# thu-nics/ViDiT-Q

Measured on AMD Instinct MI355X. Metric: denoising steps/sec (whole node), OpenSORA STDiT 16x512x512 W8A8, higher is better.
Workload: dtype int8 (W8A8 Linear, int32 acc) + fp16 attention/residual; 1 GPU; OpenSORA STDiT-XL/2 16x512x512 W8A8 (w8a8_dynamic.yaml), 1 prompt per GPU, DDIM-100 schedule, cfg 4.0, cfg_split, depth 28; prompts_in_flight=1, prompts=1, status_word=0, hip_graph=True, cond_uncond_streams=2

## Files before the change

include/viditq.h:

```cpp
#ifndef VIDITQ_H
#define VIDITQ_H

#include <stdint.h>

#ifdef __cplusplus
extern "C" {
#endif

#define VQ_OK 0
#define VQ_EINVAL (-1)
#define VQ_ESHAPE (-2)
#define VQ_ELAUNCH (-3)
#define VQ_EUNSUP (-4)

#define VQ_ST_EPSFILL 1

#define VQ_GEMM_DEFAULT (-1)

#define VQ_EPI_NONE 0
#define VQ_EPI_GELU 1
#define VQ_EPI_GATE_RESID 2
#define VQ_EPI_RESID 3

int vq_version(void);
// ... 187 lines not shown
                     int row, int n_rows, int eps_f16, int xm_f16, void* stream);

#define VQ_SA_ROW 16
#define VQ_SA_CFG 0
#define VQ_SA_SIGMA 1
#define VQ_SA_ALPHA 2
#define VQ_SA_OC 3
#define VQ_SA_CX 4
#define VQ_SA_CG0 5
#define VQ_SA_CG1 6
#define VQ_SA_CN 7
#define VQ_SA_OP 8
#define VQ_SA_PX 9
#define VQ_SA_PG0 10
#define VQ_SA_PG1 11
#define VQ_SA_PN 12
#define VQ_SA_T_NEXT 14
int vq_cfg_sa_step(const void* eps, const float* x, const float* xp, float* hist, const float* noise, const float* coef,
                   const int32_t* step, float* x_out, float* xp_out, void* x_model, int n, int C, int inner, long ld_eps,
                   int row, int n_rows, int eps_f16, int xm_f16, void* stream);

int vq_linear_f16(const void* x, const void* w, const void* bias, void* out, int M, int N, int K, long ldx, long ldw,
                  long ldo, int act_in, int act_out, void* stream);

#ifdef __cplusplus
}
#endif
#endif
```

vidit-q_amd/_lib.py:

```python
from __future__ import annotations

import ctypes as C
import os

_HERE = os.path.dirname(os.path.abspath(__file__))
LIB_PATH = os.environ.get("VIDITQ_LIB") or os.path.join(_HERE, "csrc", "libviditq_hip.so")

VQ_OK = 0
VQ_ST_EPSFILL = 1
EPI_NONE, EPI_GELU, EPI_GATE_RESID, EPI_RESID = 0, 1, 2, 3

_vp, _i, _f, _l = C.c_void_p, C.c_int, C.c_float, C.c_long

SIGNATURES = {
    "vq_version": (_i, []),
    "vq_strerror": (C.c_char_p, [_i]),
    "vq_last_hip_error": (_i, []),
    "vq_gelu_rowquant": (_i, [_vp, _vp, _vp, _vp, _vp, _vp, _vp, _i, _i, _i, _i, _i, _vp, _vp]),
    "vq_rowquant": (_i, [_vp, _vp, _i, _i, _vp, _vp, _vp, _vp, _vp, _vp, _vp, _vp, _vp, _i,
                         _i, _i, _i, _i, _i, _vp, _vp]),
    "vq_ln_modulate_rowquant": (_i, [_vp, _vp, _vp, _f, _i, _vp, _vp, _vp, _vp, _vp, _vp, _vp,
                                     _i, _i, _i, _i, _i, _vp, _vp]),
    "vq_smooth_reciprocal": (_i, [_vp, _vp, _i, _vp, _vp]),
    "vq_rowquant_smooth_multi": (_i, [_vp, _i, _vp, _vp, _vp, _vp, _vp, _vp, _i, _i, _i, _i, _vp, _vp]),
# ... 4 lines not shown
    "vq_smooth_div_check": (_i, [_vp, _vp, _vp, _vp, _l, _vp]),
    "vq_fakequant_act": (_i, [_vp, _vp, _vp, _vp, _vp, _vp, _vp, _i, _i, _i, _i, _i, _i, _vp, _vp, _vp]),
    "vq_epsfill_fixup": (_i, [_vp, _vp, _vp, _vp, _vp, _vp, _i, _i, _i, _i, _i, _vp]),
    "vq_pack_weight": (_i, [_vp, _vp, _vp, _vp, _vp, _vp, _vp, _vp, _i, _i, _i, _i, _vp]),
    "vq_weight_minmax": (_i, [_vp, _vp, _vp, _vp, _i, _i, _i, _i, _vp, _vp]),
    "vq_gemm_i8_batched": (_i, [_vp] * 10 + [_i] * 6 + [_vp]),
    "vq_gemm_i8_grouped": (_i, [_i] + [_vp] * 10 + [_i] * 6 + [_vp]),
    "vq_gemm_i8": (_i, [_vp, _vp, _vp, _vp, _vp, _vp, _vp, _vp, _vp, _vp, _i, _vp, _vp,
                        _i, _i, _i, _i, _i, _i, _i, _i, _vp]),
    "vq_gemm_i8_rowquant_static": (_i, [_vp] * 17 + [_i] * 8 + [_vp]),
    "vq_gemm_i8_cross_attn": (_i, [_vp] * 12 + [_i] * 10 + [_l] * 4 + [_vp, _f, _vp]),
    "vq_gemm_i8_stamped": (_i, [_vp] * 10 + [_i] * 5 + [_vp, _l, _vp]),
    "vq_attn_fwd": (_i, [_vp, _vp, _vp, _vp, _i, _i, _i, _i, _i, _l, _l, _l, _l, _l, _l, _vp, _f, _vp]),
    "vq_attn_fwd_route": (_i, [_vp, _vp, _vp, _vp, _i, _i, _i, _i, _i, _l, _l, _l, _l, _l, _l, _vp, _f, _vp]),
    "vq_attn_temporal": (_i, [_vp, _vp, _vp, _vp, _i, _i, _i, _i, _i, _l, _l, _f, _vp]),
    "vq_attn_temporal_rowquant": (_i, [_vp, _vp, _vp, _vp, _vp, _vp, _vp, _vp, _vp, _vp, _vp, _i, _i, _i, _i, _i, _l, _i, _f,
                                       _vp]),
    "vq_attn_temporal_rowquant_shared": (_i, [_vp] * 11 + [_i] * 5 + [_l, _i, _i, _f, _vp]),
    "vq_attn_temporal_long": (_i, [_vp] * 11 + [_i] * 5 + [_l, _l, _i, _f, _vp]),
    "vq_attn_temporal_rowquant_static": (_i, [_vp] * 12 + [_i] * 5 + [_l, _l, _i, _i, _f, _vp]),
    "vq_attn_fwd_rowquant_static": (_i, [_vp] * 12 + [_i] * 5 + [_l] * 6 + [_vp, _i, _i, _f, _vp]),
    "vq_adaln_table": (_i, [_vp, _vp, _vp, _i, _i, _i, _vp]),
    "vq_linear_f16": (_i, [_vp, _vp, _vp, _vp, _i, _i, _i, _l, _l, _l, _i, _i, _vp]),
    "vq_cfg_ddim_step": (_i, [_vp, _vp, _vp, _vp, _i, _i, _i, _f, _f, _f, _f, _f, _vp]),
    "vq_cfg_dpmpp_step": (_i, [_vp] * 7 + [_i, _i, _i, _l, _i, _i, _i, _i, _vp]),
    "vq_cfg_dpmpp_step_patch": (_i, [_vp] * 8 + [_i] * 9 + [_l] + [_i] * 5 + [_vp]),
    "vq_dpmpp_advance": (_i, [_vp, _vp, _i, _vp, _i, _vp]),
    "vq_cfg_ddpm_step": (_i, [_vp] * 8 + [_i, _i, _i, _l, _i, _i, _i, _i, _i, _vp]),
    "vq_cfg_sa_step": (_i, [_vp] * 10 + [_i, _i, _i, _l, _i, _i, _i, _i, _vp]),
}

DPMPP_ROW = 16
(DPMPP_ORDER, DPMPP_TAYLOR, DPMPP_CFG, DPMPP_SIGMA, DPMPP_ALPHA, DPMPP_INV_ALPHA, DPMPP_X, DPMPP_M0, DPMPP_D1, DPMPP_D2,
 DPMPP_INV_R0, DPMPP_INV_R1, DPMPP_R0_FRAC, DPMPP_INV_R01, DPMPP_T_NEXT) = range(15)
DDPM_ROW = 16
(DDPM_CFG, DDPM_A, DDPM_B, DDPM_C1, DDPM_C2, DDPM_MIN_LOG, DDPM_MAX_LOG, DDPM_NONZERO, DDPM_CLIP) = range(9)
DDPM_T_NEXT = 14
SA_ROW = 16
(SA_CFG, SA_SIGMA, SA_ALPHA, SA_OC, SA_CX, SA_CG0, SA_CG1, SA_CN, SA_OP, SA_PX, SA_PG0, SA_PG1, SA_PN) = range(13)
SA_T_NEXT = 14

_lib = None


class VQError(RuntimeError):
    pass
# ... 36 lines not shown
```

vidit-q_amd/csrc/fp_linear.hip:

```cpp
#include "vq_common.h"

#define FPL_NONE 0
#define FPL_SILU 1
#define FPL_GELU 2

template <int ACT>
__device__ __forceinline__ float fpl_act(float v) {
    if constexpr (ACT == FPL_SILU) {
        return v * __builtin_amdgcn_rcpf(1.0f + __builtin_amdgcn_exp2f(-1.4426950408889634f * v));
    } else if constexpr (ACT == FPL_GELU) {
        const float w = v * fmaf(v * v, -0.044715f * 2.302208198f, -2.302208198f);
        return v * __builtin_amdgcn_rcpf(1.0f + __builtin_amdgcn_exp2f(w));
    } else {
        return v;
    }
}

template <int ACT_IN, int ACT_OUT, bool SPLITK>
__global__ __launch_bounds__(256) void fp_linear_kernel(const half_t* __restrict__ x, const half_t* __restrict__ w,
                                                        const half_t* __restrict__ bias, half_t* __restrict__ out, int M,
                                                        int N, int K, long ldx, long ldw, long ldo) {
    __shared__ float red[3][64][4];
    const int lane = threadIdx.x & 63, wave = __builtin_amdgcn_readfirstlane(threadIdx.x >> 6);
    const int lq = lane & 15, g4 = lane >> 4;
// ... 22 lines not shown
            }
            acc = __builtin_amdgcn_mfma_f32_16x16x32_f16(wa[u], xa[u], acc, 0, 0, 0);
        }
    }
    if constexpr (SPLITK) {
        if (wave > 0) *reinterpret_cast<float4v*>(&red[wave - 1][lane][0]) = acc;
        __syncthreads();
        if (wave > 0) return;
#pragma unroll
        for (int p = 0; p < 3; ++p) {
            const float4v o = *reinterpret_cast<const float4v*>(&red[p][lane][0]);
            acc += o;
        }
    }
    const int m = m0 + lq, n = n0 + 4 * g4;
    if (m < M && n < N) {
        half4 o;
#pragma unroll
        for (int r = 0; r < 4; ++r) o[r] = (half_t)fpl_act<ACT_OUT>(acc[r] + (bias ? (float)bias[n + r] : 0.f));
        *reinterpret_cast<half4*>(out + (long)m * ldo + n) = o;
    }
}

template <int AI, int AO>
static void fpl_go(const half_t* x, const half_t* w, const half_t* bias, half_t* out, int M, int N, int K, long ldx, long ldw,
                   long ldo, hipStream_t st) {
    const int mt = (M + 15) / 16, nt = (N + 15) / 16;
    if (K <= 32)
        hipLaunchKernelGGL((fp_linear_kernel<AI, AO, false>), dim3((mt + 3) / 4, nt), dim3(256), 0, st, x, w, bias, out, M, N, K, ldx,
                           ldw, ldo);
    else
        hipLaunchKernelGGL((fp_linear_kernel<AI, AO, true>), dim3(mt, nt), dim3(256), 0, st, x, w, bias, out, M, N, K, ldx, ldw, ldo);
}

extern "C" int vq_linear_f16(const void* x, const void* w, const void* bias, void* out, int M, int N, int K, long ldx,
                             long ldw, long ldo, int act_in, int act_out, void* stream) {
    if (!x || !w || !out) return VQ_EINVAL;
    if (M <= 0 || N <= 0 || K <= 0) return VQ_EINVAL;
    if (K % 8 != 0 || N % 4 != 0 || ldx % 8 != 0 || ldw % 8 != 0 || ldo % 4 != 0 || ldx < K || ldw < K || ldo < N) return VQ_ESHAPE;
    if (act_in < 0 || act_in > 2 || act_out < 0 || act_out > 2) return VQ_EUNSUP;
    if ((M + 15) / 16 > 2147483647 / 4 || (N + 15) / 16 > 65535) return VQ_ESHAPE;
    const half_t* X = (const half_t*)x;
    const half_t* W = (const half_t*)w;
    const half_t* Bv = (const half_t*)bias;
    half_t* O = (half_t*)out;
    hipStream_t st = (hipStream_t)stream;
#define FPL_CASE(AI, AO) \
    if (act_in == AI && act_out == AO) fpl_go<AI, AO>(X, W, Bv, O, M, N, K, ldx, ldw, ldo, st)
    FPL_CASE(FPL_NONE, FPL_NONE);
    else FPL_CASE(FPL_NONE, FPL_SILU);
    else FPL_CASE(FPL_NONE, FPL_GELU);
    else FPL_CASE(FPL_SILU, FPL_NONE);
    else return VQ_EUNSUP;
#undef FPL_CASE
    return vq_check_launch();
}
```

vidit-q_amd/graph.py:

```python
from __future__ import annotations

import os
from typing import Dict, Hashable, Optional, Tuple

import torch


def _capture(fn, warmup: int, first=None, debug: bool = False):
    side = torch.cuda.Stream()
    side.wait_stream(torch.cuda.current_stream())
    with torch.cuda.stream(side), torch.no_grad():
        if first is not None:
            first()
            side.synchronize()
        for _ in range(warmup):
            fn()
        side.synchronize()
    torch.cuda.current_stream().wait_stream(side)
    graph = torch.cuda.CUDAGraph()
    if debug:
        graph.enable_debug_mode()
    with torch.no_grad(), torch.cuda.graph(graph, capture_error_mode="thread_local"):
        out = fn()
    return graph, out
# ... 12 lines not shown
        self.mask = mask
        self.cfg_split = bool(getattr(qnn, "cfg_split", False))
        from . import _lib
        dump = os.environ.get("VQ_GRAPH_DUMP")

        def counted():
            calls0 = _lib.CALLS[0]
            out = self._forward(timestep_id)
            self.c_abi_calls = _lib.CALLS[0] - calls0
            return out

        self.graph, (self.cond, self.uncond) = _capture(counted, warmup, debug=bool(dump),
                                                        first=lambda: self._forward(timestep_id, serial=True))
        self.dot_path = None
        if dump:
            try:
                self.dot_path = "%s.%d.dot" % (dump, id(self))
                self.graph.debug_dump(self.dot_path)
            except Exception:
                self.dot_path = None

    def _forward(self, t_id, serial=False):
        q = self.qnn
        if self.cfg_split and self.two_streams and not serial:
            cur = torch.cuda.current_stream()
            self.side.wait_stream(cur)
            with torch.cuda.stream(self.side):
                unc = q(self.x, self.t, self.yu, mask=self.mask, timestep_id=t_id)
            cond = q(self.x, self.t, self.yc, mask=self.mask, timestep_id=t_id)
            cur.wait_stream(self.side)
            return cond, unc
        if self.cfg_split:
            return (q(self.x, self.t, self.yc, mask=self.mask, timestep_id=t_id),
                    q(self.x, self.t, self.yu, mask=self.mask, timestep_id=t_id))
        n = self.x.shape[0]
        out = q(torch.cat([self.x, self.x]), torch.cat([self.t, self.t]), torch.cat([self.yc, self.yu]),
                mask=self.mask, timestep_id=t_id)
        return out[:n], out[n:]

    def run(self, x: torch.Tensor, timestep_id: int):
        self.x.copy_(x)
        self.t.fill_(int(timestep_id))
        self.graph.replay()
        return self.cond, self.uncond


# ... 280 lines not shown
```

vidit-q_amd/ops.py:

```python
from __future__ import annotations

import ctypes as C
from dataclasses import dataclass
from typing import List, Optional, Sequence

import torch

from . import _lib
from ._lib import EPI_GATE_RESID, EPI_GELU, EPI_NONE, EPI_RESID, VQError, check


def _L():
    return _lib.load()


def _stream() -> int:
    return torch.cuda.current_stream().cuda_stream


def _p(t: Optional[torch.Tensor]):
    return None if t is None else t.data_ptr()


def _req(t: torch.Tensor, dtype, name: str):
# ... 866 lines not shown
    R = torch.empty(rows, dtype=torch.int32, device=dev)
    scale = float(D) ** -0.5 if scale is None else float(scale)
    check(_L().vq_attn_fwd_rowquant_static(_p(q), _p(k), _p(v), _p(s), _p(s_rcp), _p(delta), _p(zp), _p(xq), _p(sx), _p(zx),
                                           _p(R), _p(o), n_seq, Lq, Lk, H, D, q_seq_stride, q_tok_stride, kv_seq_stride,
                                           kv_tok_stride, o_seq_stride, o_tok_stride, _p(kv_off), Kp, n_bits, scale,
                                           _stream()), "vq_attn_fwd_rowquant_static")
    return QAct(xq, sx, zx, R, Cc, n_bits)


def adaln_table(table: torch.Tensor, t0: torch.Tensor) -> torch.Tensor:
    _req(table, torch.float16, "table")
    _req(t0, torch.float16, "t0")
    J, Cc = table.shape
    B = t0.shape[0]
    assert t0.numel() == B * J * Cc
    mod = torch.empty((J, B, Cc), dtype=torch.float32, device=table.device)
    check(_L().vq_adaln_table(_p(table), _p(t0), _p(mod), B, J, Cc, _stream()), "vq_adaln_table")
    return mod


ACT_NONE, ACT_SILU, ACT_GELU = 0, 1, 2


def linear_f16(x: torch.Tensor, w: torch.Tensor, bias: Optional[torch.Tensor] = None, act_in: int = ACT_NONE,
               act_out: int = ACT_NONE) -> torch.Tensor:
    _req_rows(x, torch.float16, "x")
    _req_rows(w, torch.float16, "w")
    K = x.shape[-1]
    N = w.shape[0]
    assert w.dim() == 2 and w.shape[1] == K and w.stride(1) == 1
    x2 = x.reshape(-1, K)
    if x2.stride(1) != 1:
        x2 = x2.contiguous()
    if bias is not None:
        _req(bias, torch.float16, "bias")
        assert bias.numel() == N and bias.is_contiguous()
    M = x2.shape[0]
    out = torch.empty((M, N), dtype=torch.float16, device=x.device)
    check(_L().vq_linear_f16(_p(x2), _p(w), _p(bias), _p(out), M, N, K, x2.stride(0), w.stride(0), N, act_in, act_out,
                             _stream()), "vq_linear_f16")
    return out.reshape(*x.shape[:-1], N)


def cfg_ddim_step(cond: torch.Tensor, uncond: torch.Tensor, x: torch.Tensor, cfg: float, one_plus_k: float,
                  A: float, Bc: float, abar_prev: float, out: Optional[torch.Tensor] = None) -> torch.Tensor:
    _req(cond, torch.float32, "cond")
    _req(uncond, torch.float32, "uncond")
    _req(x, torch.float32, "x")
    n, Cc = x.shape[0], x.shape[1]
    inner = x[0, 0].numel()
    assert cond.shape[0] == n and cond.shape[1] == 2 * Cc and cond.shape == uncond.shape
    if out is None:
        out = torch.empty_like(x)
    check(_L().vq_cfg_ddim_step(_p(cond), _p(uncond), _p(x), _p(out), n, Cc, inner, float(cfg), float(one_plus_k),
                                float(A), float(Bc), float(abar_prev), _stream()), "vq_cfg_ddim_step")
    return out


def _dense_strides(shape):
    out, acc = [], 1
    for d in reversed(shape):
        out.append(acc)
        acc *= int(d)
    return tuple(reversed(out))
# ... 203 lines not shown
```

vidit-q_amd/qdiff/models/quant_model.py:

```python
from __future__ import annotations

import logging
import warnings

import torch
import torch.nn as nn

from ..quantizer.base_quantizer import ActQuantizer, BaseQuantizer, StraightThrough, WeightQuantizer
from .dit_quant_layer import QuantAttnLinearImg, QuantCrossAttnLinearImg
from .quant_block import BaseQuantBlock, get_specials
from .quant_layer import QuantLayer
from .stdit_quant_layer import QuantCrossAttnLinear, QuantSpatialAttnLinear, QuantTemporalAttnLinear

logger = logging.getLogger(__name__)


def pattern_in(text, pattern):
    patterns = pattern.split(".")
    texts = text.split(".")
    for i in range(len(texts)):
        for j in range(len(patterns)):
            if i + j >= len(texts):
                break
            if patterns[j] == "*":
# ... 213 lines not shown
            return 0
        v = int(self._status.item())
        if v & 1:
            msg = ("a dynamically quantized activation had a token with quant step < 1e-6: the reference would set "
                   "EVERY token's step to 1e-6 here (base_quantizer.py:220-222) and saturate the layer; the integer "
                   "path does not reproduce that degenerate fill - outputs of this run differ from the reference")
            if raise_on_eps:
                raise RuntimeError(msg)
            warnings.warn(msg)
        return v

    def forward(self, x, t, y, timestep_id=None, **kwargs):
        if timestep_id is None:
            timestep_id = t[0].item() if isinstance(t, torch.Tensor) else t
        if self.timestep_wise:
            self.set_timestep_for_quantizer(timestep_id)
        if timestep_id != self._cur_t:
            self.set_timestep_id_for_quantlayer(timestep_id)
            self._cur_t = timestep_id
        if x.is_cuda:
            self.status_word()
        return self.model(x, t, y, **kwargs)

    def __getattr__(self, name):
        try:
            return super().__getattr__(name)
        except AttributeError:
            return getattr(self.model, name)


def _device_of(model):
    for p in model.parameters():
        return p.device
    return torch.device("cpu")
```

vidit-q_amd/t2v/dpm_solver.py:

```python
from __future__ import annotations

from functools import partial

import torch

from ..t2i.dpm_solver import DPMSolverPP, _switch
from .iddpm import _accepts_timestep_id, model_forward_pair

_T2V_DPM_FUSED = _switch("VQ_T2V_DPM_FUSED", False)


def lower_order_final(steps: int) -> bool:
    return steps < 10


def forward_with_dpmsolver(model, x, timestep, y, **kwargs):
    return model.forward(x, timestep, y, **kwargs).chunk(2, dim=1)[0]


class VideoDPMSolverPP(DPMSolverPP):

    def __init__(self, net, condition, uncondition, cfg_scale, model_kwargs=None, cfg_split=False):
        super().__init__(partial(forward_with_dpmsolver, net), condition, uncondition, cfg_scale, model_kwargs)
        self.net, self.cfg_split = net, bool(cfg_split)
# ... 6 lines not shown
            self.model_kwargs["timestep_id"] = t_val
        if not self.cfg_split or self.cfg_scale == 1.0 or self.uncondition is None:
            return super()._noise(x, t_cont)
        t = torch.full((x.shape[0],), t_val, dtype=torch.float32, device=x.device)
        extra = {k: v for k, v in self.model_kwargs.items() if k not in ("mask", "timestep_id")}
        cond, uncond = model_forward_pair(self.net, x, t, self.condition, self.uncondition, self.model_kwargs.get("mask"),
                                          True, t_val, extra)
        return self._guide(torch.cat([uncond.chunk(2, dim=1)[0], cond.chunk(2, dim=1)[0]]))

    def _fused_wanted(self, x, method, fused):
        if fused is None:
            fused = _T2V_DPM_FUSED
        return bool(fused) and method == "multistep" and self.cfg_scale != 1.0 and self.uncondition is not None and x.is_cuda

    def _forward_patch(self, xm, t, t_val, side=None):
        kw = {k: v for k, v in self.model_kwargs.items() if k != "timestep_id"}
        if self._takes_id:
            kw["timestep_id"] = t_val
        net = self.net
        if not self.cfg_split:
            n = xm.shape[0] // 2
            out = net.forward(xm, t, self._joint_text(), patch_major=True, **kw)
            return out[:n], out[n:]
        if side is None:
            eps_c = net.forward(xm, t, self.condition, patch_major=True, **kw)
            return net.forward(xm, t, self.uncondition, patch_major=True, **kw), eps_c
        cur = torch.cuda.current_stream()
        side.wait_stream(cur)
        with torch.cuda.stream(side):
            eps_u = net.forward(xm, t, self.uncondition, patch_major=True, **kw)
        eps_c = net.forward(xm, t, self.condition, patch_major=True, **kw)
        cur.wait_stream(side)
        return eps_u, eps_c

    def _eager_eps(self, pair):
        return torch.cat([self.net.unpatchify(e).to(torch.float32).chunk(2, dim=1)[0] for e in pair])

    def _multistep_fused(self, x, ts, args, step_callback):
        from .. import ops
        from ..t2i.fused_loop import device_table, fused_loop
        n, steps, order = x.shape[0], args[0], args[1]
        copies = 1 if self.cfg_split else 2
        patch = tuple(self.net.patch_size)
        x = x.float().contiguous() if x.dtype != torch.float32 or not x.is_contiguous() else x
        xm = torch.cat([x] * copies).to(self.model_input_dtype)
        hist = torch.empty((3, x.numel()), dtype=torch.float32, device=x.device)
# ... 67 lines not shown
```

vidit-q_amd/t2v/stdit.py:

```python
from __future__ import annotations

import os
from typing import List

import numpy as np
import torch
import torch.nn as nn
import torch.nn.functional as F

from .. import ops
from ..qdiff.models.quant_block import QuantAttention
from ..qdiff.models.quant_layer import QuantLayer
from ..qdiff.quantizer.dynamic_quantizer import DynamicActQuantizer


def approx_gelu():
    return nn.GELU(approximate="tanh")


def t2i_modulate(x, shift, scale):
    return x * (1 + scale) + shift


def get_1d_sincos_pos_embed_from_grid(embed_dim, pos):
# ... 258 lines not shown
        q = self.q_linear(x).reshape(B * N, C).half().contiguous()
        kv = self.kv_linear(cond).reshape(-1, 2 * C).half().contiguous()
        lens = mask if mask is not None else [kv.shape[0] // B] * B
        off = seq_offsets(lens, x.device)
        o = self.core.cross(q, kv, off, B, N)
        return self.proj(o.reshape(B, N, C).to(dt))


def _switch(name: str, default: bool) -> bool:
    return os.environ.get(name, "1" if default else "0") != "0"


_ATTN_QUANT = _switch("VQ_ATTN_QUANT", True)
_GELU_QUANT = _switch("VQ_GELU_QUANT", True)
_STATIC_FUSED = True
_ATTN_QUANT_JOINT = _switch("VQ_ATTN_QUANT_JOINT", False)
_SMOOTH_JOINT = _switch("VQ_SMOOTH_JOINT", False)
_STATIC_ATTN_QUANT = _switch("VQ_STATIC_ATTN_QUANT", False)
_STATIC_FWD_ATTN_QUANT = _switch("VQ_STATIC_FWD_ATTN_QUANT", False)
_STATIC_GEMM_QUANT = _switch("VQ_STATIC_GEMM_QUANT", False)
_RUNNING_SMOOTH_DEVICE = _switch("VQ_RUNNING_SMOOTH_DEVICE", False)
EXACT_KV_EPS_FILL = _switch("VQ_EXACT_KV_EPS_FILL", True)
_CROSS_Q_FUSED = _switch("VQ_CROSS_Q_FUSED", True)


def _tensorwise_static(aq) -> bool:
    return not isinstance(aq, DynamicActQuantizer) and aq.delta.numel() == 1 and aq.zero_point.numel() == 1


def _same_dynamic(layers) -> bool:
    aqs = [l.act_quantizer for l in layers]
    return all(isinstance(a, DynamicActQuantizer) for a in aqs) and len({a.n_bits for a in aqs}) == 1


def _smooth_joint(layers, svs, B, add_rows=False) -> bool:
    return _SMOOTH_JOINT and B == 2 and not add_rows and all(s is not None for s in svs) and _same_dynamic(layers)


def _static_attn_quant(proj, T, H, D) -> bool:
    aq = proj.act_quantizer
    return _STATIC_ATTN_QUANT and _STATIC_FUSED and _tensorwise_static(aq) and ops.attn_temporal_static_ok(
        T, H, D, ops.pad128(H * D), aq.n_bits)


def _static_fwd_attn_quant(proj) -> bool:
    return _STATIC_FWD_ATTN_QUANT and _STATIC_FUSED and _tensorwise_static(proj.act_quantizer)
# ... 28 lines not shown
    aq = proj.act_quantizer
    return fused_call(aq.delta.float(), aq.zero_point.float(), aq.n_bits, sv)


def fused_rules(block, running=False) -> bool:
    for m in block.hot_layers():
        if not (isinstance(m, QuantLayer) and m.int_route_ok()):
            return False
        aq = m.act_quantizer
        if not isinstance(aq, DynamicActQuantizer) and aq.per_group:
            return False
        if getattr(m, "smooth_quant_running_stat", False) and not (
                running and m is block.mlp.fc2 and m.running_stat_device_ok()):
            return False
    return True


def fused_running_rules(block) -> bool:
    return fused_rules(block, running=True)


def takes_fused(block) -> bool:
    return block.fused_ok() or (_RUNNING_SMOOTH_DEVICE and block.fused_running_ok())


def _svec(layer):
    r, alpha = layer._range_and_alpha()
    return layer.smooth_vector(r, alpha)


def _range_of(layer, r):
    return layer._range_and_alpha()[0] if r is None else r


def ln_quant(x3, shift, scale, layers, svs, status):
    l0 = layers[0]
    if len(layers) > 1 and _smooth_joint(layers, svs, x3.shape[0]):
        qas = ops.rowquant_multi_shared(x3, svs, n_bits=l0.act_quantizer.n_bits, status=status, shift=shift, scale=scale,
                                        eps=1e-6)
        if qas is not None:
            return qas
    if all(isinstance(l.act_quantizer, DynamicActQuantizer) for l in layers):
        smooth = [None] if all(s is None for s in svs) else list(svs)
        return ops.ln_modulate_rowquant(x3, shift, scale, 1e-6, smooth=smooth, n_bits=l0.act_quantizer.n_bits,
                                        status=status)
    if _static_one_pass(layers, x3.shape[-1], ln=True):
# ... 13 lines not shown
            return qas
    if all(s is None for s in svs) and isinstance(aq, DynamicActQuantizer):
        return [att.q.quantize_input(x3, None, add_rows=tpe2, add_div=S)]
    if tpe2 is None and B == 1 and all(s is not None for s in svs) and _same_dynamic(layers):
        return ops.rowquant_multi(x3, svs, n_bits=aq.n_bits, status=st)
    if _static_one_pass(layers, x3.shape[-1], add_rows=tpe2 is not None):
        delta, zp = _static_grids(layers)
        return ops.rowquant_static(x3, delta, zp, n_bits=aq.n_bits, smooth=svs, add_rows=tpe2, add_div=S)
    return [l.quantize_input(x3, s, add_rows=tpe2, add_div=S) for l, s in zip(layers, svs)]


def temporal_proj_codes(att, qkv, B, T, S, sv):
    proj, aq = att.proj, att.proj.act_quantizer
    dynamic = isinstance(aq, DynamicActQuantizer)
    if _ATTN_QUANT and dynamic and aq.n_bits == 8 and (B == 1 or not _ATTN_QUANT_JOINT):
        return att.core.temporal_quantized(qkv, B, T, S, status=proj.status, s=sv)
    if _ATTN_QUANT and _ATTN_QUANT_JOINT and dynamic:
        return att.core.temporal_quantized_shared(qkv, B, T, S, aq.n_bits, status=proj.status, s=sv)
    if _static_attn_quant(proj, T, att.core.num_heads, att.core.head_dim):
        return att.core.temporal_quantized_static(qkv, B, T, S, aq.delta.float(), aq.zero_point.float(), aq.n_bits, s=sv)
    return None


def proj_into_resid(layer, r, qa, x2, gate=None, rows_per_gate=None, pw=None):
    if pw is None:
        pw = layer.packed_weight(_range_of(layer, r), _svec(layer))
    if gate is None:
        return ops.gemm_i8(qa, pw, bias=layer.bias_f32(), out=x2, epilogue=ops.EPI_RESID, resid=x2)
    return ops.gemm_i8(qa, pw, bias=layer.bias_f32(), out=x2, epilogue=ops.EPI_GATE_RESID, resid=x2, gate=gate,
                       rows_per_gate=rows_per_gate)


def attn_proj_stage(proj, r, x2, B, N, fused, plain, att_o, gate=None):
    sv = _svec(proj)
    qa = fused(sv)
    if qa is None:
        att_o = plain(att_o)
        qa = proj.quantize_input(att_o.view(B, N, -1), sv)
    proj_into_resid(proj, r, qa, x2, gate, N)
    return att_o


def _cross_q_fused_shape(H, D, K, B, N, bound=None) -> bool:
    C, Kp = H * D, (K + 127) // 128 * 128
    return D == 72 and C % 288 == 0 and N > 0 and N % 256 == 0 and 0 < K <= 16384 and B * N * Kp < 1 << 32 and \
        C * Kp < 1 << 32 and (bound is None or 0 < bound <= 128)


_CROSS_Q_FUSED_ROUND = 256


def _cross_q_fused(ca, B, N) -> bool:
    H, D = ca.core.num_heads, ca.core.head_dim
    return _CROSS_Q_FUSED and not _static_fwd_attn_quant(ca.proj) and _cross_q_fused_shape(
        H, D, ca.q_linear.in_features, B, N) and ((B * N // 256) * (H * D // 288)) % _CROSS_Q_FUSED_ROUND == 0


def cross_stage(ca, r, x2, x3, B, N, y_lens, prompt_kv, att_o):
    ql, sv = ca.q_linear, _svec(ca.q_linear)
    kv = None
    if _cross_q_fused(ca, B, N):
        kv = prompt_kv()
        core = ca.core
        C = core.num_heads * core.head_dim
        bound = int(getattr(y_lens, "max_len", 0)) or kv.shape[0]
        if _cross_q_fused_shape(core.num_heads, core.head_dim, ql.in_features, B, N, bound) and kv.stride(0) % 8 == 0:
            def fused_q(o):
                if o is None:
                    o = torch.empty((B * N, C), dtype=torch.float16, device=x3.device)
                return ops.gemm_i8_cross_attn(ql.quantize_input(x3, sv), ql.packed_weight(_range_of(ql, r), sv), ql.bias_f32(),
                                              kv, kv[:, C:], o, B, N, bound, core.num_heads, core.head_dim, 0, kv.stride(0),
                                              N * o.stride(0), o.stride(0), kv_off=y_lens, scale=core.scale)
            return attn_proj_stage(ca.proj, r, x2, B, N, lambda s: None, fused_q, att_o)
    q = ops.gemm_i8(ql.quantize_input(x3, sv), ql.packed_weight(_range_of(ql, r), sv), bias=ql.bias_f32())
    if kv is None:
        kv = prompt_kv()
    return attn_proj_stage(
        ca.proj, r, x2, B, N,
        lambda s: fwd_attn_quantized_static(ca.proj, s, lambda d, z, nb, sm: ca.core.cross_quantized_static(
            q, kv, y_lens, B, N, d, z, nb, s=sm)),
        lambda o: ca.core.cross(q, kv, y_lens, B, N, out=o), att_o)


def mlp_stage(mlp, r, x2, x3, B, N, shift, scale, gate, status):
    fc1, fc2 = mlp.fc1, mlp.fc2
    s1 = _svec(fc1)
    qa = ln_quant(x3, shift, scale, (fc1,), [s1], status)[0]
    pw1 = fc1.packed_weight(_range_of(fc1, r), s1)
    if getattr(fc2, "smooth_quant_running_stat", False):
        h = ops.gemm_i8(qa, pw1, bias=fc1.bias_f32(), epilogue=ops.EPI_GELU)
        qa, pw2 = fc2.running_stat_step(h.view(B, N, -1))
        return proj_into_resid(fc2, r, qa, x2, gate, N, pw=pw2)
    s2 = _svec(fc2)
    qa2 = mlp_quantized_static(fc1, fc2, qa, pw1, s2)
    if qa2 is None:
        one_pass = _GELU_QUANT and fc2.gelu_one_pass_ok(B, fc2.in_features, s2)
        h = ops.gemm_i8(qa, pw1, bias=fc1.bias_f32(), epilogue=ops.EPI_NONE if one_pass else ops.EPI_GELU)
        h3 = h.view(B, N, -1)
        qa2 = fc2.quantize_gelu_input(h3, s2) if one_pass else fc2.quantize_input(h3, s2)
    return proj_into_resid(fc2, r, qa2, x2, gate, N)


def prompt_kv_exact_fill(layer, y3, r, sv, pw):
    aq = layer.act_quantizer
# ... 99 lines not shown
        kkey = (y2, pw_kv.wq, ca.kv_linear.act_quantizer.n_bits)
        kv = self._kv_cache.get(kkey) if self.cache_prompt else None
        if kv is None:
            kv = prompt_kv_exact_fill(ca.kv_linear, y2.view(1, -1, C), r, sv, pw_kv)
            if self.cache_prompt:
                self._kv_cache.put(kkey, kv)
        return kv

    def _qkv_gemm(self, att, r, svs, qas, M):
        layers = (att.q, att.k, att.v)
        fused, pws = self._qkv_weights(att, r, svs)
        C = self.hidden_size
        qkv = torch.empty((M, 3 * C), dtype=torch.float16, device=qas[0].xq.device)
        if fused is not None and len(qas) == 1:
            ops.gemm_i8(qas[0], fused[0], bias=fused[1], out=qkv)
        elif len({(p.N, p.K, p.Kp, p.n_bits) for p in pws}) == 1 and len({(a.K, a.Kp) for a in qas}) == 1:
            ops.gemm_i8_grouped([qas[j if len(qas) > 1 else 0] for j in range(3)], pws, [l.bias_f32() for l in layers], out=qkv)
        else:
            for j, l in enumerate(layers):
                ops.gemm_i8(qas[j if len(qas) > 1 else 0], pws[j], bias=l.bias_f32(), out=qkv[:, j * C:(j + 1) * C])
        return qkv

    def forward_fused(self, x2, y2, t0, y_lens, tpe, B, kv_ready=None, mod=None):
        T, S, C = self.d_t, self.d_s, self.hidden_size
        N = T * S
        a1, a2 = self.attn, self.attn_temp
        r, _ = a1.q._range_and_alpha()
        if mod is None:
            mod = ops.adaln_table(self.scale_shift_table.detach(), t0.reshape(B, -1))
        shift_msa, scale_msa, gate_msa, shift_mlp, scale_mlp, gate_mlp = [mod[j] for j in range(6)]
        x3 = x2.view(B, N, C)
        st = a1.q.status
        svs = [_svec(l) for l in (a1.q, a1.k, a1.v)]
        qkv = self._qkv_gemm(a1, r, svs, ln_quant(x3, shift_msa, scale_msa, (a1.q, a1.k, a1.v), svs, st), B * N)
        att_o = attn_proj_stage(
            a1.proj, r, x2, B, N,
            lambda s: fwd_attn_quantized_static(a1.proj, s, lambda d, z, nb, sm: a1.core.spatial_quantized_static(
                qkv, B * T, S, d, z, nb, s=sm)),
            lambda o: a1.core.spatial(qkv, B * T, S), None, gate_msa)
        svs = [_svec(l) for l in (a2.q, a2.k, a2.v)]
        tpe2 = None if tpe is None else tpe.reshape(T, C).contiguous()
        qkv = self._qkv_gemm(a2, r, svs, temporal_qkv_codes(a2, x3, svs, tpe2, B, S), B * N)
        att_o = attn_proj_stage(a2.proj, r, x2, B, N, lambda s: temporal_proj_codes(a2, qkv, B, T, S, s),
                                lambda o: a2.core.temporal(qkv, B, T, S, out=o), att_o, gate_msa)
        cross_stage(self.cross_attn, r, x2, x3, B, N, y_lens,
                    lambda: kv_ready if kv_ready is not None else self.prompt_kv(y2), att_o)
        mlp_stage(self.mlp, r, x2, x3, B, N, shift_mlp, scale_mlp, gate_mlp, st)
        return x2


class STDiT(nn.Module):
    def __init__(self, input_size=(1, 32, 32), in_channels=4, patch_size=(1, 2, 2), hidden_size=1152, depth=28,
                 num_heads=16, mlp_ratio=4.0, class_dropout_prob=0.1, pred_sigma=True, drop_path=0.0,
                 no_temporal_pos_emb=False, caption_channels=4096, model_max_length=120, dtype=torch.float32,
                 space_scale=1.0, time_scale=1.0, freeze=None, enable_flashattn=True, enable_layernorm_kernel=False,
                 enable_sequence_parallelism=False, separate_qkv=True):
        super().__init__()
        assert not enable_sequence_parallelism, "sequence parallelism is training-only in the reference"
        self.pred_sigma = pred_sigma
        self.in_channels = in_channels
        self.out_channels = in_channels * 2 if pred_sigma else in_channels
        self.hidden_size, self.patch_size, self.input_size = hidden_size, patch_size, input_size
        self.num_patches = int(np.prod([input_size[i] // patch_size[i] for i in range(3)]))
        self.num_temporal = input_size[0] // patch_size[0]
        self.num_spatial = self.num_patches // self.num_temporal
        self.num_heads, self.dtype, self.depth, self.mlp_ratio = num_heads, dtype, depth, mlp_ratio
        self.no_temporal_pos_emb = no_temporal_pos_emb
        self.space_scale, self.time_scale = space_scale, time_scale
        self.separate_qkv = True

# ... 120 lines not shown
        if len(st) < 4 or st[3] is None:
            wdq = torch.stack([l.dequantized_weight_f16(0, None) for l in layers])
            bdq = torch.stack([l.bias.detach().half() for l in layers]).contiguous() if l0.bias is not None else None
            st = self._kv_stack = (st[0], st[1], st[2], (wdq, bdq))
        wdq, bdq = st[3]
        ops.epsfill_fixup(flag, y3.contiguous(), None, wdq, bdq, out, n_bits=l0.act_quantizer.n_bits)
        return [out[i] for i in range(len(layers))]

    def _prompt_tokens(self, y, mask, C):
        fcs = (self.y_embedder.y_proj.fc1, self.y_embedder.y_proj.fc2)
        fp = all(not getattr(m, "weight_quant", False) and not getattr(m, "act_quant", False) for m in fcs)
        key = None
        if self.cache_prompt and fp and not self.training:
            key = (y, mask, fcs[0].weight, fcs[1].weight)
            hit = self._prompt_cache.get(key)
            if hit is not None:
                return hit
        ye = self.y_embedder(y.to(self.dtype), self.training)
        out = self._select_prompt_tokens(ye, mask, C)
        if key is not None:
            self._prompt_cache.put(key, out)
        return out

    def forward(self, x, timestep, y, mask=None, patch_major=False):
        x = x.to(self.dtype)
        timestep = timestep.to(self.dtype)
        C = self.hidden_size
        x = self.x_embedder(x)
        B = x.shape[0]
        x = x.reshape(B, self.num_temporal, self.num_spatial, C) + self.pos_embed
        x = x.reshape(B, self.num_patches, C).contiguous()
        t = self.t_embedder(timestep, dtype=x.dtype)
        t0 = fp_edge_linear(self.t_block[1], t, act_in=ops.ACT_SILU)
        if t0 is None:
            t0 = self.t_block(t)
        y, y_lens, off = self._prompt_tokens(y, mask, C)

        fused = x.is_cuda and x.dtype == torch.float16 and all(takes_fused(b) for b in self.blocks)
        if fused:
            x2 = x.reshape(B * self.num_patches, C)
            y2 = y.reshape(-1, C).contiguous()
            if off is None:
                off = seq_offsets(y_lens, x.device)
            t0c = t0.contiguous()
            kvs = self._all_prompt_kv(y2)
            mods = self._all_adaln(t0c, B)
            for i, block in enumerate(self.blocks):
                block.forward_fused(x2, y2, t0c, off, self.pos_embed_temporal if i == 0 else None, B,
                                    kv_ready=None if kvs is None else kvs[i], mod=mods[6 * i:6 * i + 6])
            x = x2.reshape(B, self.num_patches, C)
        else:
            for i, block in enumerate(self.blocks):
                x = block(x, y, t0, y_lens, self.pos_embed_temporal if i == 0 else None)
        x = self.final_layer(x, t)
        if patch_major:
            return x
        x = self.unpatchify(x)
        return x.to(torch.float32)

    def unpatchify(self, x):
        N_t, N_h, N_w = [self.input_size[i] // self.patch_size[i] for i in range(3)]
        T_p, H_p, W_p = self.patch_size
        B = x.shape[0]
        x = x.reshape(B, N_t, N_h, N_w, T_p, H_p, W_p, self.out_channels)
        x = x.permute(0, 7, 1, 4, 2, 5, 3, 6)
        return x.reshape(B, self.out_channels, N_t * T_p, N_h * H_p, N_w * W_p)


def STDiT_XL_2(from_pretrained=None, **kwargs):
    model = STDiT(depth=28, hidden_size=1152, patch_size=(1, 2, 2), num_heads=16, **kwargs)
    if from_pretrained is not None:
        load_split_qkv(model, torch.load(from_pretrained, map_location="cpu"))
    return model


def load_split_qkv(model: STDiT, state_dict: dict):
    sd = {}
    for k, v in state_dict.items():
        if k.endswith(".qkv.weight") or k.endswith(".qkv.bias"):
            base, kind = k.rsplit(".qkv.", 1)
            for name, part in zip("qkv", v.chunk(3, dim=0)):
# ... 5 lines not shown
```

Baseline: 26.11 denoising steps/s.

## Share cond/uncond prefix up to first cross-attn and add skinny fp16 linear

Adds a forward_pair path that runs the embedding, timestep MLP, adaLN table and block 0's spatial and temporal attention once. It then forks only the prompt-dependent remainder (cross-attn onward) across the cond and uncond branches, since that earlier work does not depend on the prompt. Separately, it adds a skinny-M fp16 linear kernel (M<=16) that splits K across waves with MFMA and reduces in LDS, auto-selected for large weights such as the timestep MLP. Risks: the shared prefix assumes block 0 is calibrated and has no running statistics, and the first cross-attn's residual output is now written to a separate buffer.

```diff
diff --git a/include/viditq.h b/include/viditq.h
--- a/include/viditq.h
+++ b/include/viditq.h
@@ -233,6 +233,11 @@
 
 int vq_linear_f16(const void* x, const void* w, const void* bias, void* out, int M, int N, int K, long ldx, long ldw,
                   long ldo, int act_in, int act_out, void* stream);
+#define VQ_LINEAR_AUTO 0
+#define VQ_LINEAR_TILE 1
+#define VQ_LINEAR_SKINNY 2
+int vq_linear_f16_route(const void* x, const void* w, const void* bias, void* out, int M, int N, int K, long ldx, long ldw,
+                        long ldo, int act_in, int act_out, int route, void* stream);
 
 #ifdef __cplusplus
 }
diff --git a/vidit-q_amd/_lib.py b/vidit-q_amd/_lib.py
--- a/vidit-q_amd/_lib.py
+++ b/vidit-q_amd/_lib.py
@@ -50,6 +50,7 @@
     "vq_attn_fwd_rowquant_static": (_i, [_vp] * 12 + [_i] * 5 + [_l] * 6 + [_vp, _i, _i, _f, _vp]),
     "vq_adaln_table": (_i, [_vp, _vp, _vp, _i, _i, _i, _vp]),
     "vq_linear_f16": (_i, [_vp, _vp, _vp, _vp, _i, _i, _i, _l, _l, _l, _i, _i, _vp]),
+    "vq_linear_f16_route": (_i, [_vp, _vp, _vp, _vp, _i, _i, _i, _l, _l, _l, _i, _i, _i, _vp]),
     "vq_cfg_ddim_step": (_i, [_vp, _vp, _vp, _vp, _i, _i, _i, _f, _f, _f, _f, _f, _vp]),
     "vq_cfg_dpmpp_step": (_i, [_vp] * 7 + [_i, _i, _i, _l, _i, _i, _i, _i, _vp]),
     "vq_cfg_dpmpp_step_patch": (_i, [_vp] * 8 + [_i] * 9 + [_l] + [_i] * 5 + [_vp]),
diff --git a/vidit-q_amd/csrc/fp_linear.hip b/vidit-q_amd/csrc/fp_linear.hip
--- a/vidit-q_amd/csrc/fp_linear.hip
+++ b/vidit-q_amd/csrc/fp_linear.hip
@@ -68,6 +68,92 @@
     }
 }
 
+#define FPL_SK_TN 2
+
+template <int ACT_IN, int ACT_OUT, int NS>
+__global__ __launch_bounds__(256) void fp_linear_skinny_kernel(const half_t* __restrict__ x, const half_t* __restrict__ w,
+                                                               const half_t* __restrict__ bias, half_t* __restrict__ out, int M,
+                                                               int N, int K, long ldx, long ldw, long ldo) {
+    __shared__ float red[FPL_SK_TN][3][64][4];
+    const int lane = threadIdx.x & 63, wave = __builtin_amdgcn_readfirstlane(threadIdx.x >> 6);
+    const int lq = lane & 15, g4 = lane >> 4;
+    const int mr = lq < M ? lq : M - 1;
+    const half_t* xr = x + (long)mr * ldx + 8 * g4;
+    const half_t* wr[FPL_SK_TN];
+#pragma unroll
+    for (int j = 0; j < FPL_SK_TN; ++j) {
+        const int n0 = (blockIdx.x * FPL_SK_TN + j) * 16;
+        const int nr = n0 + lq < N ? n0 + lq : N - 1;
+        wr[j] = w + (long)nr * ldw + 8 * g4;
+    }
+    float4v acc[FPL_SK_TN];
+#pragma unroll
+    for (int j = 0; j < FPL_SK_TN; ++j) acc[j] = float4v{0.f, 0.f, 0.f, 0.f};
+    const int nst = K / 32;
+    const int nw = (nst - wave + 3) / 4;
+    for (int i0 = 0; i0 < nw; i0 += NS) {
+        half8 xa[NS], wa[FPL_SK_TN][NS];
+#pragma unroll
+        for (int u = 0; u < NS; ++u) {
+            const int i = i0 + u < nw ? i0 + u : nw - 1;
+            const long k = (long)(wave + 4 * i) * 32;
+            xa[u] = *reinterpret_cast<const half8*>(xr + k);
+#pragma unroll
+            for (int j = 0; j < FPL_SK_TN; ++j) wa[j][u] = *reinterpret_cast<const half8*>(wr[j] + k);
+        }
+#pragma unroll
+        for (int u = 0; u < NS; ++u) {
+            if (i0 + u < nw) {
+                if constexpr (ACT_IN != FPL_NONE) {
+#pragma unroll
+                    for (int e = 0; e < 8; ++e) xa[u][e] = (half_t)fpl_act<ACT_IN>((float)xa[u][e]);
+                }
+#pragma unroll
+                for (int j = 0; j < FPL_SK_TN; ++j) acc[j] = __builtin_amdgcn_mfma_f32_16x16x32_f16(wa[j][u], xa[u], acc[j], 0, 0, 0);
+            }
+        }
+    }
+    if (wave > 0) {
+#pragma unroll
+        for (int j = 0; j < FPL_SK_TN; ++j) *reinterpret_cast<float4v*>(&red[j][wave - 1][lane][0]) = acc[j];
+    }
+    __syncthreads();
+    if (wave > 0) return;
+#pragma unroll
+    for (int j = 0; j < FPL_SK_TN; ++j) {
+#pragma unroll
+        for (int p = 0; p < 3; ++p) {
+            const float4v o = *reinterpret_cast<const float4v*>(&red[j][p][lane][0]);
+            acc[j] += o;
+        }
+        const int m = lq, n = (blockIdx.x * FPL_SK_TN + j) * 16 + 4 * g4;
+        if (m < M && n < N) {
+            half4 o;
+#pragma unroll
+            for (int r = 0; r < 4; ++r) o[r] = (half_t)fpl_act<ACT_OUT>(acc[j][r] + (bias ? (float)bias[n + r] : 0.f));
+            *reinterpret_cast<half4*>(out + (long)m * ldo + n) = o;
+        }
+    }
+}
+
+static bool fpl_skinny_shape(int M, int K) { return M <= 16 && K % 32 == 0 && K >= 128; }
+
+#define FPL_SK_AUTO_MIN_WEIGHT (4L << 20)
+static bool fpl_skinny_auto(int M, int N, int K) { return fpl_skinny_shape(M, K) && (long)N * K >= FPL_SK_AUTO_MIN_WEIGHT; }
+
+template <int AI, int AO>
+static void fpl_go_skinny(const half_t* x, const half_t* w, const half_t* bias, half_t* out, int M, int N, int K, long ldx,
+                          long ldw, long ldo, hipStream_t st) {
+    const int nt = (N + 15) / 16, nw = (K / 32 + 3) / 4;
+    const dim3 grid((nt + FPL_SK_TN - 1) / FPL_SK_TN), block(256);
+    if (nw <= 2)
+        hipLaunchKernelGGL((fp_linear_skinny_kernel<AI, AO, 2>), grid, block, 0, st, x, w, bias, out, M, N, K, ldx, ldw, ldo);
+    else if (nw <= 9)
+        hipLaunchKernelGGL((fp_linear_skinny_kernel<AI, AO, 9>), grid, block, 0, st, x, w, bias, out, M, N, K, ldx, ldw, ldo);
+    else
+        hipLaunchKernelGGL((fp_linear_skinny_kernel<AI, AO, 12>), grid, block, 0, st, x, w, bias, out, M, N, K, ldx, ldw, ldo);
+}
+
 template <int AI, int AO>
 static void fpl_go(const half_t* x, const half_t* w, const half_t* bias, half_t* out, int M, int N, int K, long ldx, long ldw,
                    long ldo, hipStream_t st) {
@@ -79,25 +165,36 @@
         hipLaunchKernelGGL((fp_linear_kernel<AI, AO, true>), dim3(mt, nt), dim3(256), 0, st, x, w, bias, out, M, N, K, ldx, ldw, ldo);
 }
 
-extern "C" int vq_linear_f16(const void* x, const void* w, const void* bias, void* out, int M, int N, int K, long ldx,
-                             long ldw, long ldo, int act_in, int act_out, void* stream) {
+extern "C" int vq_linear_f16_route(const void* x, const void* w, const void* bias, void* out, int M, int N, int K, long ldx,
+                                   long ldw, long ldo, int act_in, int act_out, int route, void* stream) {
     if (!x || !w || !out) return VQ_EINVAL;
     if (M <= 0 || N <= 0 || K <= 0) return VQ_EINVAL;
     if (K % 8 != 0 || N % 4 != 0 || ldx % 8 != 0 || ldw % 8 != 0 || ldo % 4 != 0 || ldx < K || ldw < K || ldo < N) return VQ_ESHAPE;
     if (act_in < 0 || act_in > 2 || act_out < 0 || act_out > 2) return VQ_EUNSUP;
+    if (route < VQ_LINEAR_AUTO || route > VQ_LINEAR_SKINNY) return VQ_EUNSUP;
     if ((M + 15) / 16 > 2147483647 / 4 || (N + 15) / 16 > 65535) return VQ_ESHAPE;
+    if (route == VQ_LINEAR_SKINNY && !fpl_skinny_shape(M, K)) return VQ_EUNSUP;
+    const bool skinny = route == VQ_LINEAR_SKINNY || (route == VQ_LINEAR_AUTO && fpl_skinny_auto(M, N, K));
     const half_t* X = (const half_t*)x;
     const half_t* W = (const half_t*)w;
     const half_t* Bv = (const half_t*)bias;
     half_t* O = (half_t*)out;
     hipStream_t st = (hipStream_t)stream;
-#define FPL_CASE(AI, AO) \
-    if (act_in == AI && act_out == AO) fpl_go<AI, AO>(X, W, Bv, O, M, N, K, ldx, ldw, ldo, st)
-    FPL_CASE(FPL_NONE, FPL_NONE);
-    else FPL_CASE(FPL_NONE, FPL_SILU);
-    else FPL_CASE(FPL_NONE, FPL_GELU);
-    else FPL_CASE(FPL_SILU, FPL_NONE);
+#define FPL_CASE(AI, AO)                                                            \
+    if (act_in == AI && act_out == AO) {                                            \
+        if (skinny) fpl_go_skinny<AI, AO>(X, W, Bv, O, M, N, K, ldx, ldw, ldo, st); \
+        else fpl_go<AI, AO>(X, W, Bv, O, M, N, K, ldx, ldw, ldo, st);               \
+    }
+    FPL_CASE(FPL_NONE, FPL_NONE)
+    else FPL_CASE(FPL_NONE, FPL_SILU)
+    else FPL_CASE(FPL_NONE, FPL_GELU)
+    else FPL_CASE(FPL_SILU, FPL_NONE)
     else return VQ_EUNSUP;
 #undef FPL_CASE
     return vq_check_launch();
 }
+
+extern "C" int vq_linear_f16(const void* x, const void* w, const void* bias, void* out, int M, int N, int K, long ldx,
+                             long ldw, long ldo, int act_in, int act_out, void* stream) {
+    return vq_linear_f16_route(x, w, bias, out, M, N, K, ldx, ldw, ldo, act_in, act_out, VQ_LINEAR_AUTO, stream);
+}
diff --git a/vidit-q_amd/graph.py b/vidit-q_amd/graph.py
--- a/vidit-q_amd/graph.py
+++ b/vidit-q_amd/graph.py
@@ -58,6 +58,9 @@
 
     def _forward(self, t_id, serial=False):
         q = self.qnn
+        if self.cfg_split and hasattr(q, "forward_pair"):
+            side = self.side if self.two_streams and not serial else None
+            return q.forward_pair(self.x, self.t, self.yc, self.yu, mask=self.mask, timestep_id=t_id, side=side)
         if self.cfg_split and self.two_streams and not serial:
             cur = torch.cuda.current_stream()
             self.side.wait_stream(cur)
diff --git a/vidit-q_amd/ops.py b/vidit-q_amd/ops.py
--- a/vidit-q_amd/ops.py
+++ b/vidit-q_amd/ops.py
@@ -912,8 +912,10 @@
 ACT_NONE, ACT_SILU, ACT_GELU = 0, 1, 2
 
 
-def linear_f16(x: torch.Tensor, w: torch.Tensor, bias: Optional[torch.Tensor] = None, act_in: int = ACT_NONE,
-               act_out: int = ACT_NONE) -> torch.Tensor:
+LINEAR_AUTO, LINEAR_TILE, LINEAR_SKINNY = 0, 1, 2
+
+
+def _linear_f16(x, w, bias, act_in, act_out, route):
     _req_rows(x, torch.float16, "x")
     _req_rows(w, torch.float16, "w")
     K = x.shape[-1]
@@ -927,9 +929,23 @@
         assert bias.numel() == N and bias.is_contiguous()
     M = x2.shape[0]
     out = torch.empty((M, N), dtype=torch.float16, device=x.device)
-    check(_L().vq_linear_f16(_p(x2), _p(w), _p(bias), _p(out), M, N, K, x2.stride(0), w.stride(0), N, act_in, act_out,
-                             _stream()), "vq_linear_f16")
+    if route == LINEAR_AUTO:
+        check(_L().vq_linear_f16(_p(x2), _p(w), _p(bias), _p(out), M, N, K, x2.stride(0), w.stride(0), N, act_in, act_out,
+                                 _stream()), "vq_linear_f16")
+    else:
+        check(_L().vq_linear_f16_route(_p(x2), _p(w), _p(bias), _p(out), M, N, K, x2.stride(0), w.stride(0), N, act_in,
+                                       act_out, route, _stream()), "vq_linear_f16_route")
     return out.reshape(*x.shape[:-1], N)
+
+
+def linear_f16(x: torch.Tensor, w: torch.Tensor, bias: Optional[torch.Tensor] = None, act_in: int = ACT_NONE,
+               act_out: int = ACT_NONE) -> torch.Tensor:
+    return _linear_f16(x, w, bias, act_in, act_out, LINEAR_AUTO)
+
+
+def linear_f16_route(x: torch.Tensor, w: torch.Tensor, bias: Optional[torch.Tensor] = None, act_in: int = ACT_NONE,
+                     act_out: int = ACT_NONE, route: int = LINEAR_AUTO) -> torch.Tensor:
+    return _linear_f16(x, w, bias, act_in, act_out, route)
 
 
 def cfg_ddim_step(cond: torch.Tensor, uncond: torch.Tensor, x: torch.Tensor, cfg: float, one_plus_k: float,
diff --git a/vidit-q_amd/qdiff/models/quant_model.py b/vidit-q_amd/qdiff/models/quant_model.py
--- a/vidit-q_amd/qdiff/models/quant_model.py
+++ b/vidit-q_amd/qdiff/models/quant_model.py
@@ -259,6 +259,22 @@
             self.status_word()
         return self.model(x, t, y, **kwargs)
 
+    def forward_pair(self, x, t, y_cond, y_uncond, timestep_id=None, side=None, **kwargs):
+        if timestep_id is None:
+            timestep_id = t[0].item() if isinstance(t, torch.Tensor) else t
+        pair = getattr(self.model, "forward_pair", None)
+        if pair is None:
+            from ...t2v.stdit import run_pair
+            return run_pair(lambda y: self.forward(x, t, y, timestep_id=timestep_id, **kwargs), y_cond, y_uncond, side)
+        if self.timestep_wise:
+            self.set_timestep_for_quantizer(timestep_id)
+        if timestep_id != self._cur_t:
+            self.set_timestep_id_for_quantlayer(timestep_id)
+            self._cur_t = timestep_id
+        if x.is_cuda:
+            self.status_word()
+        return pair(x, t, y_cond, y_uncond, side=side, **kwargs)
+
     def __getattr__(self, name):
         try:
             return super().__getattr__(name)
diff --git a/vidit-q_amd/t2v/dpm_solver.py b/vidit-q_amd/t2v/dpm_solver.py
--- a/vidit-q_amd/t2v/dpm_solver.py
+++ b/vidit-q_amd/t2v/dpm_solver.py
@@ -52,6 +52,9 @@
             n = xm.shape[0] // 2
             out = net.forward(xm, t, self._joint_text(), patch_major=True, **kw)
             return out[:n], out[n:]
+        if hasattr(net, "forward_pair"):
+            eps_c, eps_u = net.forward_pair(xm, t, self.condition, self.uncondition, patch_major=True, side=side, **kw)
+            return eps_u, eps_c
         if side is None:
             eps_c = net.forward(xm, t, self.condition, patch_major=True, **kw)
             return net.forward(xm, t, self.uncondition, patch_major=True, **kw), eps_c
diff --git a/vidit-q_amd/t2v/stdit.py b/vidit-q_amd/t2v/stdit.py
--- a/vidit-q_amd/t2v/stdit.py
+++ b/vidit-q_amd/t2v/stdit.py
@@ -304,6 +304,7 @@
 _RUNNING_SMOOTH_DEVICE = _switch("VQ_RUNNING_SMOOTH_DEVICE", False)
 EXACT_KV_EPS_FILL = _switch("VQ_EXACT_KV_EPS_FILL", True)
 _CROSS_Q_FUSED = _switch("VQ_CROSS_Q_FUSED", True)
+_PAIR_SHARED = _switch("VQ_PAIR_SHARED", True)
 
 
 def _tensorwise_static(aq) -> bool:
@@ -378,6 +379,35 @@
 
 def takes_fused(block) -> bool:
     return block.fused_ok() or (_RUNNING_SMOOTH_DEVICE and block.fused_running_ok())
+
+
+def _pair_fused(model) -> bool:
+    return all(takes_fused(b) for b in model.blocks) and model.blocks[0].fused_ok()
+
+
+def _pair_no_running_stat(block) -> bool:
+    return not any(getattr(m, "smooth_quant_running_stat", False) for m in block.hot_layers())
+
+
+def _pair_calibrated(block) -> bool:
+    return all(isinstance(m, QuantLayer) and m.int_route_ok() for m in block.hot_layers())
+
+
+def pair_shared_ok(model, x) -> bool:
+    return bool(_PAIR_SHARED and x.is_cuda and model.dtype == torch.float16 and not model.training and len(model.blocks) > 0
+                and _pair_fused(model) and _pair_no_running_stat(model.blocks[0]) and _pair_calibrated(model.blocks[0]))
+
+
+def run_pair(chain, y_cond, y_uncond, side=None):
+    if side is None:
+        return chain(y_cond), chain(y_uncond)
+    cur = torch.cuda.current_stream()
+    side.wait_stream(cur)
+    with torch.cuda.stream(side):
+        unc = chain(y_uncond)
+    cond = chain(y_cond)
+    cur.wait_stream(side)
+    return cond, unc
 
 
 def _svec(layer):
@@ -437,22 +467,24 @@
     return None
 
 
-def proj_into_resid(layer, r, qa, x2, gate=None, rows_per_gate=None, pw=None):
+def proj_into_resid(layer, r, qa, x2, gate=None, rows_per_gate=None, pw=None, out=None):
     if pw is None:
         pw = layer.packed_weight(_range_of(layer, r), _svec(layer))
+    if out is None:
+        out = x2
     if gate is None:
-        return ops.gemm_i8(qa, pw, bias=layer.bias_f32(), out=x2, epilogue=ops.EPI_RESID, resid=x2)
-    return ops.gemm_i8(qa, pw, bias=layer.bias_f32(), out=x2, epilogue=ops.EPI_GATE_RESID, resid=x2, gate=gate,
+        return ops.gemm_i8(qa, pw, bias=layer.bias_f32(), out=out, epilogue=ops.EPI_RESID, resid=x2)
+    return ops.gemm_i8(qa, pw, bias=layer.bias_f32(), out=out, epilogue=ops.EPI_GATE_RESID, resid=x2, gate=gate,
                        rows_per_gate=rows_per_gate)
 
 
-def attn_proj_stage(proj, r, x2, B, N, fused, plain, att_o, gate=None):
+def attn_proj_stage(proj, r, x2, B, N, fused, plain, att_o, gate=None, out=None):
     sv = _svec(proj)
     qa = fused(sv)
     if qa is None:
         att_o = plain(att_o)
         qa = proj.quantize_input(att_o.view(B, N, -1), sv)
-    proj_into_resid(proj, r, qa, x2, gate, N)
+    proj_into_resid(proj, r, qa, x2, gate, N, out=out)
     return att_o
 
 
@@ -471,8 +503,15 @@
         H, D, ca.q_linear.in_features, B, N) and ((B * N // 256) * (H * D // 288)) % _CROSS_Q_FUSED_ROUND == 0
 
 
-def cross_stage(ca, r, x2, x3, B, N, y_lens, prompt_kv, att_o):
+def cross_q_codes(ca, x3):
+    return ca.q_linear.quantize_input(x3, _svec(ca.q_linear))
+
+
+def cross_stage(ca, r, x2, x3, B, N, y_lens, prompt_kv, att_o, qa=None, out=None):
     ql, sv = ca.q_linear, _svec(ca.q_linear)
+
+    def codes():
+        return qa if qa is not None else ql.quantize_input(x3, sv)
     kv = None
     if _cross_q_fused(ca, B, N):
         kv = prompt_kv()
@@ -483,18 +522,18 @@
             def fused_q(o):
                 if o is None:
                     o = torch.empty((B * N, C), dtype=torch.float16, device=x3.device)
-                return ops.gemm_i8_cross_attn(ql.quantize_input(x3, sv), ql.packed_weight(_range_of(ql, r), sv), ql.bias_f32(),
+                return ops.gemm_i8_cross_attn(codes(), ql.packed_weight(_range_of(ql, r), sv), ql.bias_f32(),
                                               kv, kv[:, C:], o, B, N, bound, core.num_heads, core.head_dim, 0, kv.stride(0),
                                               N * o.stride(0), o.stride(0), kv_off=y_lens, scale=core.scale)
-            return attn_proj_stage(ca.proj, r, x2, B, N, lambda s: None, fused_q, att_o)
-    q = ops.gemm_i8(ql.quantize_input(x3, sv), ql.packed_weight(_range_of(ql, r), sv), bias=ql.bias_f32())
+            return attn_proj_stage(ca.proj, r, x2, B, N, lambda s: None, fused_q, att_o, out=out)
+    q = ops.gemm_i8(codes(), ql.packed_weight(_range_of(ql, r), sv), bias=ql.bias_f32())
     if kv is None:
         kv = prompt_kv()
     return attn_proj_stage(
         ca.proj, r, x2, B, N,
         lambda s: fwd_attn_quantized_static(ca.proj, s, lambda d, z, nb, sm: ca.core.cross_quantized_static(
             q, kv, y_lens, B, N, d, z, nb, s=sm)),
-        lambda o: ca.core.cross(q, kv, y_lens, B, N, out=o), att_o)
+        lambda o: ca.core.cross(q, kv, y_lens, B, N, out=o), att_o, out=out)
 
 
 def mlp_stage(mlp, r, x2, x3, B, N, shift, scale, gate, status):
@@ -640,13 +679,17 @@
         return qkv
 
     def forward_fused(self, x2, y2, t0, y_lens, tpe, B, kv_ready=None, mod=None):
+        return self.fused_rest(self.fused_prefix(x2, t0, tpe, B, mod=mod), x2, y2, y_lens, B, kv_ready=kv_ready)
+
+    def fused_prefix(self, x2, t0, tpe, B, mod=None, cross_q=False):
         T, S, C = self.d_t, self.d_s, self.hidden_size
         N = T * S
         a1, a2 = self.attn, self.attn_temp
         r, _ = a1.q._range_and_alpha()
         if mod is None:
             mod = ops.adaln_table(self.scale_shift_table.detach(), t0.reshape(B, -1))
-        shift_msa, scale_msa, gate_msa, shift_mlp, scale_mlp, gate_mlp = [mod[j] for j in range(6)]
+        gate_msa = mod[2]
+        shift_msa, scale_msa = mod[0], mod[1]
         x3 = x2.view(B, N, C)
         st = a1.q.status
         svs = [_svec(l) for l in (a1.q, a1.k, a1.v)]
@@ -661,9 +704,20 @@
         qkv = self._qkv_gemm(a2, r, svs, temporal_qkv_codes(a2, x3, svs, tpe2, B, S), B * N)
         att_o = attn_proj_stage(a2.proj, r, x2, B, N, lambda s: temporal_proj_codes(a2, qkv, B, T, S, s),
                                 lambda o: a2.core.temporal(qkv, B, T, S, out=o), att_o, gate_msa)
+        return r, mod, att_o, cross_q_codes(self.cross_attn, x3) if cross_q else None
+
+    def fused_rest(self, prefix, x2, y2, y_lens, B, kv_ready=None, out=None):
+        T, S, C = self.d_t, self.d_s, self.hidden_size
+        N = T * S
+        r, mod, att_o, qa = prefix
+        shift_mlp, scale_mlp, gate_mlp = mod[3], mod[4], mod[5]
+        x3 = x2.view(B, N, C)
         cross_stage(self.cross_attn, r, x2, x3, B, N, y_lens,
-                    lambda: kv_ready if kv_ready is not None else self.prompt_kv(y2), att_o)
-        mlp_stage(self.mlp, r, x2, x3, B, N, shift_mlp, scale_mlp, gate_mlp, st)
+                    lambda: kv_ready if kv_ready is not None else self.prompt_kv(y2), None if out is not None else att_o,
+                    qa=qa, out=out)
+        if out is not None:
+            x2, x3 = out, out.view(B, N, C)
+        mlp_stage(self.mlp, r, x2, x3, B, N, shift_mlp, scale_mlp, gate_mlp, self.attn.q.status)
         return x2
 
 
@@ -830,7 +884,7 @@
             self._prompt_cache.put(key, out)
         return out
 
-    def forward(self, x, timestep, y, mask=None, patch_major=False):
+    def _head(self, x, timestep):
         x = x.to(self.dtype)
         timestep = timestep.to(self.dtype)
         C = self.hidden_size
@@ -842,6 +896,19 @@
         t0 = fp_edge_linear(self.t_block[1], t, act_in=ops.ACT_SILU)
         if t0 is None:
             t0 = self.t_block(t)
+        return x, t, t0
+
+    def _tail(self, x, t, patch_major):
+        x = self.final_layer(x, t)
+        if patch_major:
+            return x
+        x = self.unpatchify(x)
+        return x.to(torch.float32)
+
+    def forward(self, x, timestep, y, mask=None, patch_major=False):
+        C = self.hidden_size
+        x, t, t0 = self._head(x, timestep)
+        B = x.shape[0]
         y, y_lens, off = self._prompt_tokens(y, mask, C)
 
         fused = x.is_cuda and x.dtype == torch.float16 and all(takes_fused(b) for b in self.blocks)
@@ -860,11 +927,37 @@
         else:
             for i, block in enumerate(self.blocks):
                 x = block(x, y, t0, y_lens, self.pos_embed_temporal if i == 0 else None)
-        x = self.final_layer(x, t)
-        if patch_major:
-            return x
-        x = self.unpatchify(x)
-        return x.to(torch.float32)
+        return self._tail(x, t, patch_major)
+
+    def forward_pair(self, x, timestep, y_cond, y_uncond, mask=None, patch_major=False, side=None):
+        if not pair_shared_ok(self, x):
+            return run_pair(lambda y: self.forward(x, timestep, y, mask=mask, patch_major=patch_major), y_cond, y_uncond, side)
+        C, P = self.hidden_size, self.num_patches
+
+        def prompt(y):
+            y, y_lens, off = self._prompt_tokens(y, mask, C)
+            y2 = y.reshape(-1, C).contiguous()
+            if off is None:
+                off = seq_offsets(y_lens, x.device)
+            return y2, off, self._all_prompt_kv(y2)
+
+        xs, t, t0 = self._head(x, timestep)
+        B = xs.shape[0]
+        x2 = xs.reshape(B * P, C)
+        t0c = t0.contiguous()
+        mods = self._all_adaln(t0c, B)
+        prefix = self.blocks[0].fused_prefix(x2, t0c, self.pos_embed_temporal, B, mod=mods[0:6], cross_q=True)
+
+        def chain(y):
+            y2, off, kvs = prompt(y)
+            xc = torch.empty_like(x2)
+            self.blocks[0].fused_rest(prefix, x2, y2, off, B, kv_ready=None if kvs is None else kvs[0], out=xc)
+            for i in range(1, len(self.blocks)):
+                self.blocks[i].forward_fused(xc, y2, t0c, off, None, B, kv_ready=None if kvs is None else kvs[i],
+                                             mod=mods[6 * i:6 * i + 6])
+            return self._tail(xc.reshape(B, P, C), t, patch_major)
+
+        return run_pair(chain, y_cond, y_uncond, side)
 
     def unpatchify(self, x):
         N_t, N_h, N_w = [self.input_size[i] // self.patch_size[i] for i in range(3)]
```

After: 26.37 denoising steps/s (median of 6 runs). Within noise of the previous version (+1.0%).
